# jwcalder/GraphLearningLayer

Hardware: AMD Instinct MI355X
Metric: GLL fwd+bwd calls/sec (base=500,batch=500,d=512,k=10) at 1/2/4/8 GPU (higher is better)
Workload: dtype f32; 1 GPU; ns; base=500, batch=500, d=512, k=10, classes=10, parallelism=dp1, upstream_grad=fixed seeded dL/dU, autograd_thread=caller, collective=none

## Files before the change

graphlearninglayer_amd/_lib.py:

```python
from __future__ import annotations

import ctypes as ct
import os
import threading

HERE = os.path.dirname(os.path.abspath(__file__))
LIB_PATH = os.environ.get("GLL_LIB_PATH") or os.path.join(HERE, "libgll.so")

GLL_OK = 0
GLL_DT_F32, GLL_DT_F64, GLL_DT_I64 = 0, 1, 2
FLAG_CG_GRID = 1
FLAG_CG_PERCOL = 8
FLAG_DIAG_GRID_OVERSUB = 128
FLAG_DIAG_GRID_FAIL = 256
FLAG_CG_ELL = 512
FLAG_CG_VR = 1024
FLAG_GRAD_ROWS = 2048
FLAG_GRAD_CHUNK = 4096
FLAG_GRAM_INLINE = 8192
FLAG_BWD_UNFUSED = 16384
FLAG_KNN_PANEL = 65536
FLAG_D2_F32 = 131072
FLAG_ROW_ORDER_OFF = 262144
KNOB_VR_RV, KNOB_GRID_CAP, KNOB_GRAM_TILE, KNOB_SEL_FORM, KNOB_GRAM_TAIL, KNOB_ROW_PRE = 0, 1, 2, 3, 4, 5
KNOB_GRAD_SPLIT = 6
ST_TINY_EPS, ST_FWD_NONCONV, ST_FWD_ITERS, ST_BWD_NONCONV, ST_BWD_ITERS = 0, 1, 2, 3, 4
ST_KNN_RESCAN = 5
ST_SOLVE_FAILED = 6
ST_GRID_RESCUED = 10
ST_KNN_MERGE = 7
ST_GRAD_SPLIT = 12
ST_NWORDS = 16
K_GRAM, K_SELECT, K_FINALIZE, K_CG, K_EDGE, K_GRAD = range(6)
K_BWD = 6
K_PARAM = 7
K_LOSS = 8
K_COUNT = 9
PG_Y, PG_TAU, PG_EPS = 1, 2, 4
SCORE_NONE, SCORE_ENTROPY, SCORE_L2 = 0, 1, 2
XT_F32, XT_F16, XT_BF16 = 0, 1, 2
UF_NORMALIZE = 1
MAX_D_FEATURES = 4096

EXPORTS = (
    "gll_workspace_bytes", "gll_forward", "gll_backward", "gll_forward_batched",
    "gll_backward_batched", "gll_param_grad_scratch_bytes", "gll_param_grad_batched",
    "gll_ce_head_scratch_bytes", "gll_ce_head_batched", "gll_margin_head_scratch_bytes",
    "gll_margin_head_batched", "gll_graph", "gll_workspace_view",
    "gll_cg_csr_workspace_bytes", "gll_cg_csr", "gll_prof_enable", "gll_prof_read",
    "gll_kernel_name", "gll_strerror", "gll_set_knob", "gll_build_id", "gll_select_route",
    "gll_workspace_solve_view", "gll_workspace_knn_view", "gll_gram_route",
    "gll_features_forward", "gll_features_backward", "gll_features_calls", "gll_fused_plan",
    "gll_objective_head_scratch_bytes", "gll_objective_head_batched",
)


class Problem(ct.Structure):
    _fields_ = [
        ("n", ct.c_int32), ("d", ct.c_int32), ("base", ct.c_int32), ("C", ct.c_int32),
        ("K", ct.c_int32), ("max_iter", ct.c_int32), ("tau", ct.c_float), ("eps", ct.c_float),
        ("rtol", ct.c_float), ("flags", ct.c_int32), ("status_sink", ct.c_void_p),
    ]


class View(ct.Structure):
    _fields_ = [(name, ct.c_void_p) for name in (
        "knn_idx", "knn_d2", "eps", "row_start", "row_len", "col", "w", "d2", "deg", "U32",
        "wadj", "status")]


class SolveView(ct.Structure):
    _fields_ = [(name, ct.c_void_p) for name in ("ucnt", "diag", "rhs", "P", "ell", "vr")] + [
        (name, ct.c_int32) for name in ("SE", "VRM", "Wcap", "RCAP")]


class KnnView(ct.Structure):
    _fields_ = [(name, ct.c_void_p) for name in (
        "D2", "d2_scale", "xhi", "xlo", "xnrm", "pid", "perm")] + [("plane_stride", ct.c_int64)] + [
        (name, ct.c_int32) for name in ("planes", "ldD", "rows", "d2_half", "dp", "order")]


GRAM_ROUTE_WORDS = 9
GRAM_BF3, GRAM_BF3H, GRAM_BF3S, GRAM_BF3W, GRAM_PK, GRAM_PK2 = range(6)

_lock = threading.Lock()
_lib = None


def _declare(lib):
    P = ct.POINTER(Problem)
    vp, i32, sz = ct.c_void_p, ct.c_int, ct.c_size_t
    lib.gll_workspace_bytes.argtypes = [P]
    lib.gll_workspace_bytes.restype = sz
    lib.gll_forward.argtypes = [P, vp, vp, i32, vp, vp, vp]
    lib.gll_forward.restype = i32
    lib.gll_backward.argtypes = [P, vp, vp, i32, vp, vp, i32, vp, vp]
    lib.gll_backward.restype = i32
    lib.gll_forward_batched.argtypes = [P, i32, vp, vp, i32, vp, vp, vp]
    lib.gll_forward_batched.restype = i32
    lib.gll_backward_batched.argtypes = [P, i32, vp, vp, vp, i32, vp, vp]
    lib.gll_backward_batched.restype = i32
    lib.gll_param_grad_scratch_bytes.argtypes = [P, i32]
    lib.gll_param_grad_scratch_bytes.restype = sz
    lib.gll_param_grad_batched.argtypes = [P, i32, vp, i32, vp, vp, vp, vp, vp]
    lib.gll_param_grad_batched.restype = i32
    lib.gll_ce_head_scratch_bytes.argtypes = [P, i32]
    lib.gll_ce_head_scratch_bytes.restype = sz
    lib.gll_ce_head_batched.argtypes = [P, i32, vp, vp, vp, vp, vp, vp, vp, vp, vp]
    lib.gll_ce_head_batched.restype = i32
    lib.gll_margin_head_scratch_bytes.argtypes = [P, i32]
    lib.gll_margin_head_scratch_bytes.restype = sz
    lib.gll_margin_head_batched.argtypes = [P, i32, vp, vp, vp, vp, vp, vp, vp, vp, vp, vp]
    lib.gll_margin_head_batched.restype = i32
    lib.gll_objective_head_scratch_bytes.argtypes = [P, i32]
    lib.gll_objective_head_scratch_bytes.restype = sz
    f64 = ct.c_double
    lib.gll_objective_head_batched.argtypes = [P, i32, vp, vp, f64, f64, f64, vp, vp, vp, vp, vp,
                                               vp, vp, i32, vp, ct.c_int64, vp, vp, vp]
    lib.gll_objective_head_batched.restype = i32
    lib.gll_graph.argtypes = [P, vp, vp, vp]
    lib.gll_graph.restype = i32
    lib.gll_workspace_view.argtypes = [P, vp, ct.POINTER(View)]
    lib.gll_workspace_view.restype = i32
    lib.gll_workspace_solve_view.argtypes = [P, vp, ct.POINTER(SolveView)]
    lib.gll_workspace_solve_view.restype = i32
    lib.gll_workspace_knn_view.argtypes = [P, i32, vp, ct.POINTER(KnnView)]
    lib.gll_workspace_knn_view.restype = i32
    lib.gll_gram_route.argtypes = [P, i32, i32, i32, ct.POINTER(ct.c_int32)]
    lib.gll_gram_route.restype = i32
    lib.gll_cg_csr_workspace_bytes.argtypes = [i32, i32]
    lib.gll_cg_csr_workspace_bytes.restype = sz
    lib.gll_cg_csr.argtypes = [i32, i32, vp, vp, vp, vp, vp, ct.c_float, i32, vp, vp, vp, vp]
    lib.gll_cg_csr.restype = i32
    lib.gll_prof_enable.argtypes = [i32, i32]
    lib.gll_prof_enable.restype = i32
    lib.gll_prof_read.argtypes = [i32, ct.POINTER(ct.c_double), ct.POINTER(ct.c_int)]
    lib.gll_prof_read.restype = i32
    lib.gll_kernel_name.argtypes = [i32]
    lib.gll_kernel_name.restype = ct.c_char_p
    lib.gll_select_route.argtypes = [ct.POINTER(Problem), i32, i32, i32, ct.POINTER(ct.c_int32)]
    lib.gll_select_route.restype = i32
    lib.gll_fused_plan.argtypes = [ct.POINTER(Problem), i32, i32, ct.POINTER(ct.c_int32)]
    lib.gll_fused_plan.restype = i32
    lib.gll_set_knob.argtypes = [i32, i32]
    lib.gll_set_knob.restype = i32
    lib.gll_strerror.argtypes = [i32]
    lib.gll_strerror.restype = ct.c_char_p
    lib.gll_build_id.argtypes = []
    lib.gll_build_id.restype = ct.c_char_p
    lib.gll_features_forward.argtypes = [ct.c_int64, ct.c_int32, vp, i32, i32, vp, vp, vp]
    lib.gll_features_forward.restype = i32
    lib.gll_features_backward.argtypes = [ct.c_int64, ct.c_int32, vp, vp, vp, i32, vp, i32, vp]
    lib.gll_features_backward.restype = i32
    lib.gll_features_calls.argtypes = []
    lib.gll_features_calls.restype = ct.c_int64
    return lib


def build_id() -> str:
    return lib().gll_build_id().decode()


def lib():
    global _lib
    if _lib is None:
        with _lock:
            if _lib is None:
                if not os.path.exists(LIB_PATH):
                    raise RuntimeError(
                        f"{LIB_PATH} is missing: build the HIP extension first "
                        "(python graphlearninglayer_amd/build.py). There is no CPU fallback.")
                _lib = _declare(ct.CDLL(LIB_PATH))
    return _lib


def check(rc: int, what: str):
    if rc != GLL_OK:
        raise RuntimeError(f"{what} failed: {lib().gll_strerror(rc).decode()} (code {rc})")


def kernel_name(kid: int) -> str:
    return lib().gll_kernel_name(kid).decode()
# ... 15 lines not shown
```

graphlearninglayer_amd/csrc/api.hip:

```cpp
#include <atomic>
#include <cstdio>
#include <cstdlib>
#include <mutex>
#include <unordered_map>
#include <vector>

#include "knn_route.h"

namespace gll {

struct ProfState {
    int period[GLL_K_COUNT] = {};
    long count[GLL_K_COUNT] = {};
    bool on[GLL_K_COUNT] = {};
    std::vector<hipEvent_t> pending[GLL_K_COUNT];
    std::vector<hipEvent_t> pool;
    std::mutex mu;
    hipEvent_t get() {
        if (!pool.empty()) {
            hipEvent_t e = pool.back();
            pool.pop_back();
            return e;
        }
        hipEvent_t e;
// ... 415 lines not shown
    out->diag = L.at<float>(ws, L.diag);
    out->rhs = L.at<float>(ws, L.rhs);
    out->P = L.at<float>(ws, L.P);
    out->ell = L.at<int32_t>(ws, L.ell);
    out->vr = L.at<char>(ws, L.vr);
    out->SE = ell_emit(L, 1);
    out->VRM = L.VRM;
    out->Wcap = L.Wcap;
    out->RCAP = L.RCAP;
    return GLL_OK;
}

int gll_workspace_knn_view(const gll_problem* p, int B, void* ws, gll_knn_view* out) {
    int rc = check(p);
    if (rc != GLL_OK) return rc;
    if (B < 1 || B > 65535 || !ws || !out) return GLL_ERR_INVALID_ARG;
    Layout L(*p);
    if (L.PR < L.n && B > 1) return GLL_ERR_UNSUPPORTED;
    Batch bt;
    bt.B = B;
    out->D2 = L.at<float>(ws, L.D2);
    out->d2_scale = L.at<float>(ws, L.d2s);
    out->xhi = L.at<char>(ws, L.xhi);
    out->xlo = L.at<char>(ws, L.xlo);
    out->xnrm = L.at<float>(ws, L.xnrm);
    out->pid = L.at<int32_t>(ws, L.pid);
    out->perm = L.at<int32_t>(ws, L.perm);
    out->plane_stride = int64_t(L.n) * L.ldD;
    out->planes = gram_planes(L, B);
    out->ldD = L.ldD;
    out->rows = L.PR;
    out->d2_half = d2_half(L, bt);
    out->dp = L.dp;
    out->order = locality_order(L, bt);
    return GLL_OK;
}

int gll_gram_route(const gll_problem* p, int B, int x_aligned, int cus,
                   int32_t out[GLL_GRAM_ROUTE_WORDS]) {
    int rc = check(p);
    if (rc != GLL_OK) return rc;
    if (B < 1 || B > 65535 || cus < 1 || !out) return GLL_ERR_INVALID_ARG;
    Layout L(*p);
    if (L.PR < L.n && B > 1) return GLL_ERR_UNSUPPORTED;
    Batch bt;
    bt.B = B;
    const GramRoute rt = gram_route(L, bt, x_aligned && p->d % 4 == 0, cus);
    const int32_t words[GLL_GRAM_ROUTE_WORDS] = {rt.family, rt.vec, rt.planes, rt.presplit, rt.H,
                                                 rt.t256,   rt.tail, rt.sub,   rt.panels};
    for (int q = 0; q < GLL_GRAM_ROUTE_WORDS; ++q) out[q] = words[q];
    return GLL_OK;
}

int gll_cg_csr(int m, int C, const int32_t* row_ptr, const int32_t* col, const float* val,
               const float* b, float* x, float atol, int max_iter, int32_t* iters,
               int32_t* nonconv, void* workspace, void* stream) {
    if (m < 1 || C < 1 || !row_ptr || !col || !val || !b || !x) return GLL_ERR_INVALID_ARG;
    if (m > 2048 && C <= 16) {
        if (!workspace) return GLL_ERR_INVALID_ARG;
        prof_begin(GLL_K_CG, static_cast<hipStream_t>(stream));
        const hipError_t e = launch_cg_grid_csr(m, C, row_ptr, col, val, -1, b, x,
                                                atol, max_iter > 0 ? max_iter : 100000, iters,
                                                nonconv, nullptr,
                                                static_cast<float*>(workspace),
                                                static_cast<hipStream_t>(stream));
        prof_end(GLL_K_CG, static_cast<hipStream_t>(stream));
        if (e != hipErrorNotSupported) return hip_status(e);
    }
    return hip_status(launch_cg_csr(m, C, row_ptr, col, val, b, x, atol,
                                    max_iter > 0 ? max_iter : 100000, iters, nonconv,
                                    static_cast<float*>(workspace),
                                    static_cast<hipStream_t>(stream)));
}

size_t gll_cg_csr_workspace_bytes(int m, int C) {
    const size_t per_col = size_t(5) * m * C, grid = grid_cg_workspace_floats(m, C);
    return (per_col > grid ? per_col : grid) * sizeof(float);
}

int gll_set_knob(int id, int value) {
    if (id < 0 || id >= GLL_KNOB_COUNT || value < 0) return GLL_ERR_INVALID_ARG;
    g_knobs[id].store(value, std::memory_order_relaxed);
    return GLL_OK;
}

int gll_prof_enable(int kid, int period) {
    if (kid < 0 || kid >= GLL_K_COUNT || period < 0) return GLL_ERR_INVALID_ARG;
    std::lock_guard<std::mutex> lk(g_prof.mu);
    g_prof.on[kid] = period > 0;
    g_prof.period[kid] = period > 0 ? period : 1;
    g_prof.count[kid] = 0;
    if (g_armed.kid == kid) g_armed = ArmedLaunch{};
    return GLL_OK;
}

int gll_prof_read(int kid, double* ms_total, int* count) {
    if (kid < 0 || kid >= GLL_K_COUNT || !ms_total || !count) return GLL_ERR_INVALID_ARG;
    std::lock_guard<std::mutex> lk(g_prof.mu);
    auto& v = g_prof.pending[kid];
    double tot = 0.0;
    int cnt = 0;
    for (size_t q = 0; q + 1 < v.size(); q += 2) {
        if (hipEventSynchronize(v[q + 1]) != hipSuccess) return GLL_ERR_HIP;
        float ms = 0.f;
        if (hipEventElapsedTime(&ms, v[q], v[q + 1]) != hipSuccess) return GLL_ERR_HIP;
        tot += ms;
// ... 129 lines not shown
```

graphlearninglayer_amd/csrc/gram.hip:

```cpp
#include "knn_route.h"

namespace gll {

GLL_TRACE_UNIT(knn)

typedef __bf16 bf16x8 __attribute__((ext_vector_type(8)));
typedef __bf16 bf16x4 __attribute__((ext_vector_type(4)));

__device__ __forceinline__ void shift_to_graph(const float* __restrict__& X, float* __restrict__& D2,
                                               int32_t* __restrict__& status,
                                               int32_t* __restrict__& rev_cnt, size_t xs,
                                               size_t wss) {
    X = gshift_br(X, xs);
    D2 = gshift_br(D2, wss);
    status = gshift_br(status, wss);
    rev_cnt = gshift_br(rev_cnt, wss);
}

template <int NT>
__device__ __forceinline__ void reset_call_counters(int32_t* __restrict__ status,
                                                    int32_t* __restrict__ rev_cnt, int n) {
    const int g = bx() * NT + threadIdx.x;
    if (g < kStWords) status[g] = 0;
    for (int q = g; q < n; q += gridDim.x * NT) rev_cnt[q] = 0;
}

__device__ __forceinline__ void mfma3(f32x16& acc, const __bf16* smem_h, int plane, int oa, int ob) {
    const bf16x8 ha = *reinterpret_cast<const bf16x8*>(smem_h + oa);
    const bf16x8 la = *reinterpret_cast<const bf16x8*>(smem_h + plane + oa);
    const bf16x8 hb = *reinterpret_cast<const bf16x8*>(smem_h + ob);
    const bf16x8 lb = *reinterpret_cast<const bf16x8*>(smem_h + plane + ob);
    acc = __builtin_amdgcn_mfma_f32_32x32x16_bf16(la, hb, acc, 0, 0, 0);
    acc = __builtin_amdgcn_mfma_f32_32x32x16_bf16(ha, lb, acc, 0, 0, 0);
    acc = __builtin_amdgcn_mfma_f32_32x32x16_bf16(ha, hb, acc, 0, 0, 0);
}

template <bool H>
__device__ __forceinline__ void dput(float* D2, size_t o, float v, float s) {
    if constexpr (H) reinterpret_cast<_Float16*>(D2)[o] = static_cast<_Float16>(v * s);
    else D2[o] = v;
}
template <bool H>
__device__ __forceinline__ void dput4(float* D2, size_t o, f32x4 v, float s) {
    if constexpr (H) {
        const h16x4 hv = {static_cast<_Float16>(v.x * s), static_cast<_Float16>(v.y * s),
                          static_cast<_Float16>(v.z * s), static_cast<_Float16>(v.w * s)};
        *reinterpret_cast<h16x4*>(reinterpret_cast<_Float16*>(D2) + o) = hv;
    } else {
        *reinterpret_cast<f32x4*>(D2 + o) = v;
    }
}
constexpr int kBP = 256;
constexpr int kMaxCen = 4096;
constexpr int kBS = kBP + 8;

template <int NT = 1024, typename NF>
__device__ __forceinline__ void bf3_epilogue(const f32x16& acc, const float (&sq)[8], float* smem,
                                             float (*sqp)[16], float* nrm, NF nrm_of, int bi,
                                             int bj, int n, float* __restrict__ D2, int ld,
                                             float* __restrict__ Dz) {
    static_assert(NT == 1024 || NT == 512, "bf3_epilogue: 1024- or 512-thread tiles");
    constexpr int KQ = NT / 256;
    constexpr int EP = 4096 / NT;
    constexpr int CPR = 64 / EP;
    const int tid = threadIdx.x;
    const int lane = lane_id();
    const int w = __builtin_amdgcn_readfirstlane(tid >> 6);
    const int r = lane & 31, h = lane >> 5;
    const int qd = w & 3, kq = w >> 2;
    if constexpr (NT == 1024) {
#pragma unroll
        for (int s = 0; s < 8; ++s) {
            const float t = wave_sum_dpp(sq[s]);
            if (lane == 0) sqp[s][w] = t;
        }
    } else {
#pragma unroll
        for (int s = 0; s < 8; ++s) {
            float t = dpp_add<0xB1, 0xf>(sq[s]);
            t = dpp_add<0x4E, 0xf>(t);
            t = dpp_add<0x141, 0xf>(t);
            t = dpp_add<0x140, 0xf>(t);
            t = dpp_add<0x142, 0xa>(t);
            if ((lane & 31) == 31) sqp[s][2 * w + h] = t;
        }
    }
    __syncthreads();
    float* pw = smem + (kq * 4 + qd) * 32 * 33;
#pragma unroll
    for (int e = 0; e < 16; ++e) pw[((e & 3) + 8 * (e >> 2) + 4 * h) * 33 + r] = acc[e];
    if (tid < 128) nrm[tid] = nrm_of(tid);
    __syncthreads();
    const int ti = tid / CPR, tj = EP * (tid % CPR);
    float v[EP];
    {
        const int q = 2 * (ti >> 5) + (tj >> 5), rr = ti & 31;
#pragma unroll
        for (int e = 0; e < EP; ++e) {
            const int cc = (tj & 31) + e;
            float t = 0.f;
#pragma unroll
            for (int k4 = 0; k4 < KQ; ++k4) t += smem[(k4 * 4 + q) * 32 * 33 + rr * 33 + cc];
            v[e] = t;
        }
    }
    __syncthreads();
    float* tile = smem + KQ * 4 * 32 * 33;
#pragma unroll
    for (int e = 0; e < EP; ++e) tile[ti * 65 + tj + e] = nrm[ti] + nrm[64 + tj + e] - 2.f * v[e];
    __syncthreads();
    const int i = bi * 64 + ti;
    if (i < n) {
#pragma unroll
        for (int c = 0; c < EP; c += 4) {
            float o[4];
#pragma unroll
            for (int e = 0; e < 4; ++e) {
                const int jj = tj + c + e;
                o[e] = (bi == bj && jj < ti) ? tile[jj * 65 + ti] : tile[ti * 65 + jj];
            }
            const int j0 = bj * 64 + tj + c;
            float* dst = D2 + size_t(i) * ld + j0;
            float* dz = Dz ? Dz + size_t(i) * ld + j0 : nullptr;
            if (j0 + 4 <= n) {
                __builtin_nontemporal_store(f32x4{o[0], o[1], o[2], o[3]}, reinterpret_cast<f32x4*>(dst));
                if (dz) __builtin_nontemporal_store(f32x4{0.f, 0.f, 0.f, 0.f}, reinterpret_cast<f32x4*>(dz));
            } else {
#pragma unroll
                for (int e = 0; e < 4; ++e)
                    if (j0 + e < n) {
                        dst[e] = o[e];
                        if (dz) dz[e] = 0.f;
                    }
            }
        }
    }
    const int jr = bj * 64 + ti;
    if (bi != bj && jr < n) {
#pragma unroll
        for (int c = 0; c < EP; c += 4) {
            float o[4];
#pragma unroll
            for (int e = 0; e < 4; ++e) o[e] = tile[(tj + c + e) * 65 + ti];
            const int j0 = bi * 64 + tj + c;
            float* dst = D2 + size_t(jr) * ld + j0;
            if (j0 + 4 <= n) {
                __builtin_nontemporal_store(f32x4{o[0], o[1], o[2], o[3]}, reinterpret_cast<f32x4*>(dst));
            } else {
#pragma unroll
                for (int e = 0; e < 4; ++e)
                    if (j0 + e < n) dst[e] = o[e];
            }
        }
    }
}

template <bool VEC>
__global__ __launch_bounds__(1024) void gram_bf3_kernel(const float* __restrict__ X, int n, int d,
                                                        int T, float* __restrict__ D2, int ld,
                                                        int32_t* __restrict__ status,
                                                        int32_t* __restrict__ rev_cnt,
                                                        size_t xs, size_t wss) {
    GLL_TRACE_SCOPE(4);
    GLL_TRACE_PT(10);
    shift_to_graph(X, D2, status, rev_cnt, xs, wss);
    constexpr int kPlane = 128 * kBS;
    __shared__ __attribute__((aligned(16))) __bf16 smem_h[2 * kPlane];
    __shared__ float sqp[8][16];
    __shared__ float nrm[128];
    __shared__ __attribute__((aligned(16))) float cen[kMaxCen];
    float* smem = reinterpret_cast<float*>(smem_h);
    const int tid = threadIdx.x;
    const int lane = lane_id();
    const int w = __builtin_amdgcn_readfirstlane(tid >> 6);
    const int r = lane & 31, h = lane >> 5;
    int bi = 0, rem = xcd_tile(bx(), gridDim.x);
    while (rem >= T - bi) {
        rem -= T - bi;
        ++bi;
    }
    const int bj = bi + rem;
    reset_call_counters<1024>(status, rev_cnt, n);
    const int fo = 4 * lane;
    auto slot_row = [&](int s) {
        const int R = 16 * s + w;
        const int row = (R < 64 ? bi * 64 + R : bj * 64 + R - 64);
        return X + size_t(row < n ? row : n - 1) * d;
    };
    const int nph = (d + kBP - 1) / kBP;
    f32x16 acc;
#pragma unroll
    for (int e = 0; e < 16; ++e) acc[e] = 0.f;
    float sq[8];
#pragma unroll
    for (int s = 0; s < 8; ++s) sq[s] = 0.f;
    const int qd = w & 3, kq = w >> 2;
    const int qa = qd >> 1, qb = qd & 1;

    auto gload = [&](int ph, f32x4 (&v)[8]) {
        const int k = ph * kBP + fo;
#pragma unroll
        for (int s = 0; s < 8; ++s) v[s] = load4_raw<VEC>(slot_row(s), k, d);
    };
    auto phase = [&](int ph, const f32x4 (&v)[8]) {
        const int k = ph * kBP + fo;
        __syncthreads();
        const f32x4 c = *reinterpret_cast<const f32x4*>(cen + ph * kBP + fo);
// ... 62 lines not shown
    const int lane = lane_id();
    const int w = __builtin_amdgcn_readfirstlane(tid >> 6);
    const int r = lane & 31, h = lane >> 5;
    int bi = 0, rem = xcd_tile(bx(), gridDim.x);
    while (rem >= T - bi) {
        rem -= T - bi;
        ++bi;
    }
    const int bj = bi + rem;
    reset_call_counters<512>(status, rev_cnt, n);
    const int fo = 4 * r;
    const f32x4 c = load4_raw<VEC>(X, fo, d);
    f32x4 v[8];
#pragma unroll
    for (int s = 0; s < 8; ++s) {
        const int R = 16 * s + 2 * w + h;
        const int row = R < 64 ? bi * 64 + R : bj * 64 + R - 64;
        v[s] = load4_raw<VEC>(X + size_t(row < n ? row : n - 1) * d, fo, d);
    }
    float sq[8];
#pragma unroll
    for (int s = 0; s < 8; ++s) {
        const f32x4 f = mask4<VEC>(v[s] - c, fo, d);
        sq[s] = f.x * f.x + f.y * f.y + f.z * f.z + f.w * f.w;
        bf16x4 hv, lv;
#pragma unroll
        for (int e = 0; e < 4; ++e) {
            const __bf16 hb = static_cast<__bf16>(f[e]);
            hv[e] = hb;
            lv[e] = static_cast<__bf16>(f[e] - static_cast<float>(hb));
        }
        const int o = (16 * s + 2 * w + h) * kHS + fo;
        *reinterpret_cast<bf16x4*>(smem_h + o) = hv;
        *reinterpret_cast<bf16x4*>(smem_h + kPlane + o) = lv;
    }
    __syncthreads();
    f32x16 acc;
#pragma unroll
    for (int e = 0; e < 16; ++e) acc[e] = 0.f;
    const int qd = w & 3, kq = w >> 2;
    const int qa = qd >> 1, qb = qd & 1;
#pragma unroll
    for (int st = 0; st < 4; ++st) {
        const int kk = 64 * kq + 16 * st + 8 * h;
        const int oa = (32 * qa + r) * kHS + kk, ob = (64 + 32 * qb + r) * kHS + kk;
        mfma3(acc, smem_h, kPlane, oa, ob);
    }
    bf3_epilogue<512>(acc, sq, smem, sqp, nrm, [&](int t) { return sqp[t >> 4][t & 15]; }, bi, bj,
                      n, D2, ld, nullptr);
}

template <bool VEC>
__global__ __launch_bounds__(1024) void gram_bf3s_kernel(const float* __restrict__ X, int n,
                                                         int d, int T, float* __restrict__ D2,
                                                         int ld, size_t plane,
                                                         int32_t* __restrict__ status,
                                                         int32_t* __restrict__ rev_cnt,
                                                         size_t xs, size_t wss) {
    shift_to_graph(X, D2, status, rev_cnt, xs, wss);
    constexpr int kPlane = 128 * kBS;
    __shared__ __attribute__((aligned(16))) __bf16 smem_h[2 * kPlane];
    __shared__ float sqp[8][16];
    __shared__ float nrm[128];
    float* smem = reinterpret_cast<float*>(smem_h);
    const int tid = threadIdx.x;
    const int lane = lane_id();
    const int w = __builtin_amdgcn_readfirstlane(tid >> 6);
    const int r = lane & 31, h = lane >> 5;
    const int b = xcd_tile(bx(), gridDim.x);
    const bool dg = b < T;
    int bi = b, bj = b, half = 0;
    if (!dg) {
        int rem = (b - T) >> 1;
        half = (b - T) & 1;
        bi = 0;
        while (rem >= T - 1 - bi) {
            rem -= T - 1 - bi;
            ++bi;
        }
        bj = bi + 1 + rem;
    }
    reset_call_counters<1024>(status, rev_cnt, n);
    const int fo = 4 * lane;
    f32x4 v[8];
#pragma unroll
    for (int s = 0; s < 8; ++s) {
        const int R = dg ? 16 * (s & 3) + w : 16 * s + w;
        const int row = R < 64 ? bi * 64 + R : bj * 64 + R - 64;
        const int k = (dg ? (s >> 2) : half) * kBP + fo;
        v[s] = load4_raw<VEC>(X + size_t(row < n ? row : n - 1) * d, k, d);
    }
    const f32x4 cen0 = load4_raw<VEC>(X, (dg ? 0 : half) * kBP + fo, d);
    const f32x4 cen1 = load4_raw<VEC>(X, (dg ? 1 : half) * kBP + fo, d);
    float sq[8];
#pragma unroll
    for (int s = 0; s < 8; ++s) {
        const int k = (dg ? (s >> 2) : half) * kBP + fo;
        const f32x4 f = mask4<VEC>(v[s] - (s >= 4 ? cen1 : cen0), k, d);
        sq[s] = f.x * f.x + f.y * f.y + f.z * f.z + f.w * f.w;
        bf16x4 hv, lv;
#pragma unroll
        for (int e = 0; e < 4; ++e) {
            const __bf16 hb = static_cast<__bf16>(f[e]);
            hv[e] = hb;
            lv[e] = static_cast<__bf16>(f[e] - static_cast<float>(hb));
        }
        const int o = (16 * s + w) * kBS + fo;
        *reinterpret_cast<bf16x4*>(smem_h + o) = hv;
        *reinterpret_cast<bf16x4*>(smem_h + kPlane + o) = lv;
    }
    __syncthreads();
    f32x16 acc;
#pragma unroll
    for (int e = 0; e < 16; ++e) acc[e] = 0.f;
    const int qd = w & 3, kq = w >> 2;
    const int qa = qd >> 1, qb = qd & 1;
#pragma unroll
    for (int st = 0; st < 4; ++st) {
        const int kk = 64 * kq + 16 * st + 8 * h;
        if (dg) {
            mfma3(acc, smem_h, kPlane, (32 * qa + r) * kBS + kk, (32 * qb + r) * kBS + kk);
            mfma3(acc, smem_h, kPlane, (64 + 32 * qa + r) * kBS + kk, (64 + 32 * qb + r) * kBS + kk);
        } else {
            mfma3(acc, smem_h, kPlane, (32 * qa + r) * kBS + kk, (64 + 32 * qb + r) * kBS + kk);
        }
    }
    if (dg)
        bf3_epilogue(acc, sq, smem, sqp, nrm,
                     [&](int t) {
                         const int u = t & 63;
                         return sqp[u >> 4][u & 15] + sqp[(u >> 4) + 4][u & 15];
                     },
                     bi, bj, n, D2, ld, D2 + plane);
    else
        bf3_epilogue(acc, sq, smem, sqp, nrm, [&](int t) { return sqp[t >> 4][t & 15]; }, bi, bj,
                     n, D2 + size_t(half) * plane, ld, nullptr);
}

constexpr int kWP = 128;
constexpr int kWS = kWP + 8;

template <bool VEC>
__global__ __launch_bounds__(1024) void gram_bf3w_kernel(const float* __restrict__ X, int n,
                                                         int d, int T, float* __restrict__ D2,
                                                         int ld, int32_t* __restrict__ status,
                                                         int32_t* __restrict__ rev_cnt,
                                                         size_t xs, size_t wss, int r0,
                                                         int pt) {
    shift_to_graph(X, D2, status, rev_cnt, xs, wss);
    constexpr int kPlane = 256 * kWS;
    __shared__ __attribute__((aligned(16))) __bf16 smem_h[2 * kPlane];
    __shared__ float nrm[256];
    __shared__ __attribute__((aligned(16))) float cen[kMaxCen];
    float* smem = reinterpret_cast<float*>(smem_h);
    const int tid = threadIdx.x;
    const int lane = lane_id();
    const int w = __builtin_amdgcn_readfirstlane(tid >> 6);
    const int r = lane & 31, h = lane >> 5;
    int bi = 0, rem = xcd_tile(bx(), gridDim.x), bj;
    if (pt > 0) {
        bi = (r0 >> 7) + rem / T;
        bj = rem % T;
    } else {
        while (rem >= T - bi) {
            rem -= T - bi;
            ++bi;
        }
        bj = bi + rem;
    }
    if (r0 == 0) reset_call_counters<1024>(status, rev_cnt, n);
    const int fo = 4 * (tid & 31);
    const int rs = tid >> 5;
    auto slot_row = [&](int s) {
        const int R = 32 * s + rs;
        const int row = (R < 128 ? bi * 128 + R : bj * 128 + R - 128);
        return X + size_t(row < n ? row : n - 1) * d;
    };
    const int nph = (d + kWP - 1) / kWP;
    const int sa = w >> 2, sb = w & 3;
    f32x16 acc;
#pragma unroll
    for (int e = 0; e < 16; ++e) acc[e] = 0.f;
    float sq = 0.f;

    auto gload = [&](int ph, f32x4 (&v)[8]) {
        const int k = ph * kWP + fo;
#pragma unroll
        for (int q = 0; q < 8; ++q) v[q] = load4_raw<VEC>(slot_row(q), k, d);
    };
// ... 530 lines not shown
        return;
    }
#pragma unroll
    for (int a = 0; a < 2; ++a) {
        const int ti0 = wr * 64 + a * 32;
        const int i0 = bi * 256 + ti0;
        float ni[16];
#pragma unroll
        for (int e = 0; e < 16; ++e) {
            const int i = i0 + (e & 3) + 8 * (e >> 2) + 4 * h;
            ni[e] = nrm[i < n ? i : n - 1];
        }
#pragma unroll
        for (int b = 0; b < 4; ++b) {
            const int tj = wc * 128 + b * 32 + r;
            const int j = bj * 256 + tj;
            if (diag && wc * 128 + b * 32 + 31 < ti0) continue;
            const float nj = nrm[j < n ? j : n - 1];
            float dv[16];
#pragma unroll
            for (int e = 0; e < 16; ++e) dv[e] = ni[e] + nj - 2.f * acc[a][b][e];
#pragma unroll
            for (int e = 0; e < 16; ++e) {
                const int ti = ti0 + (e & 3) + 8 * (e >> 2) + 4 * h;
                const int i = bi * 256 + ti;
                if (i < n && j < n && (!diag || tj >= ti)) dput<H>(D2, size_t(i) * ld + j, dv[e], dsc);
            }
            if (j < n) {
#pragma unroll
                for (int gq = 0; gq < 4; ++gq) {
                    const int ti = ti0 + 8 * gq + 4 * h;
                    const int i = bi * 256 + ti;
                    const size_t o = size_t(j) * ld + i;
                    if (i + 4 <= n && (!diag || tj >= ti + 3)) {
                        dput4<H>(D2, o, f32x4{dv[4 * gq], dv[4 * gq + 1], dv[4 * gq + 2], dv[4 * gq + 3]}, dsc);
                    } else {
#pragma unroll
                        for (int t = 0; t < 4; ++t)
                            if (i + t < n && (!diag || tj >= ti + t)) dput<H>(D2, o + t, dv[4 * gq + t], dsc);
                    }
                }
            }
        }
    }
}

hipError_t launch_gram(const Layout& L, const Batch& bt, void* ws, const float* X, bool vec,
                       hipStream_t s) {
    float* D2 = L.at<float>(ws, L.D2);
    int32_t* st = L.at<int32_t>(ws, L.status);
    int32_t* rc = L.at<int32_t>(ws, L.rev_cnt);
    const GramRoute rt = gram_route(L, bt, vec, device_cus());
    if (rt.panels) return hipErrorInvalidValue;
    prof_begin(GLL_K_GRAM, s);
    switch (rt.family) {
    case kGramBf3s: {
        const int T = (L.n + 63) / 64;
        const dim3 grid(T * T, bt.B);
        const size_t plane = size_t(L.n) * L.ldD;
        launch_k(rt.vec ? gram_bf3s_kernel<true> : gram_bf3s_kernel<false>, grid, 1024, 0, s, X,
                 L.n, L.d, T, D2, L.ldD, plane, st, rc, bt.x, bt.ws);
        prof_end(GLL_K_GRAM, s);
        return launch_status("gram.hip:launch_gram(bf3s)");
    }
    case kGramPk:
    case kGramPk2: {
        __bf16* Ph = L.at<__bf16>(ws, L.xhi);
        __bf16* Pl = L.at<__bf16>(ws, L.xlo);
        float* nrm = L.at<float>(ws, L.xnrm);
        const bool H = rt.H;
        const int T = (L.n + 127) / 128, T2 = (L.n + 255) / 256;
        const int64_t nt2 = int64_t(bt.B) * T2 * (T2 + 1) / 2;
        const int64_t tail = rt.tail;
        prof_span(tail > 0 ? 3 : 2);
        const dim3 sgrid((L.n + 3) / 4, bt.B);
        float* d2s = L.at<float>(ws, L.d2s);
        launch_k(rt.vec ? gram_split_kernel<true> : gram_split_kernel<false>, sgrid, 256, 0, s, X,
                 L.n, L.d, L.dp, Ph, Pl, nrm, st, rc, bt.x, bt.ws);
        if (rt.t256) {
            launch_k(H ? gram_pk2_kernel<true> : gram_pk2_kernel<false>,
                     dim3(unsigned(nt2 - tail)), 512, 0, s, Ph, Pl, nrm, L.n, L.dp, T2, D2,
                     L.ldD, bt.ws, d2s);
            if (tail > 0 && rt.sub == 4)
                launch_k(H ? gram_pk_kernel<true, 128> : gram_pk_kernel<false, 128>,
                         dim3(unsigned(4 * tail)), 256, 0, s, Ph, Pl, nrm, L.n, L.dp, T, D2, L.ldD,
                         bt.ws, d2s, int(nt2 - tail));
            else if (tail > 0)
                launch_k(H ? gram_pk_kernel<true, 64> : gram_pk_kernel<false, 64>,
                         dim3(unsigned(16 * tail)), 256, 0, s, Ph, Pl, nrm, L.n, L.dp,
                         (L.n + 63) / 64, D2, L.ldD, bt.ws, d2s, int(nt2 - tail));
        } else {
            launch_k(H ? gram_pk_kernel<true, 128> : gram_pk_kernel<false, 128>,
                     dim3(unsigned(bt.B * T * (T + 1) / 2)), 256, 0, s, Ph, Pl, nrm, L.n, L.dp, T,
                     D2, L.ldD, bt.ws, d2s, -1);
        }
        prof_end(GLL_K_GRAM, s);
        return launch_status("gram.hip:launch_gram(pk)");
    }
    case kGramBf3w: {
        const int T = (L.n + 127) / 128;
        const dim3 grid(T * (T + 1) / 2, bt.B);
        launch_k(rt.vec ? gram_bf3w_kernel<true> : gram_bf3w_kernel<false>, grid, 1024, 0, s, X,
                 L.n, L.d, T, D2, L.ldD, st, rc, bt.x, bt.ws, 0, 0);
        prof_end(GLL_K_GRAM, s);
        return launch_status("gram.hip:launch_gram(bf3w)");
    }
    case kGramBf3h: {
        const int T64 = (L.n + 63) / 64;
        const dim3 grid(T64 * (T64 + 1) / 2, bt.B);
        launch_k(rt.vec ? gram_bf3h_kernel<true> : gram_bf3h_kernel<false>, grid, 512, 0, s, X,
                 L.n, L.d, T64, D2, L.ldD, st, rc, bt.x, bt.ws);
        prof_end(GLL_K_GRAM, s);
        return launch_status("gram.hip:launch_gram(bf3h)");
    }
// ... 29 lines not shown
```

graphlearninglayer_amd/csrc/knn_route.h:

```cpp
#pragma once

#include "gll_internal.h"

namespace gll {

typedef _Float16 h16x4 __attribute__((ext_vector_type(4)));
typedef __attribute__((address_space(3))) void lds_void;

__device__ __forceinline__ int xcd_tile(int b, int nt) {
    const int x = b & 7, q = b >> 3;
    const int per = nt >> 3, extra = nt & 7;
    return x * per + (x < extra ? x : extra) + q;
}

constexpr int kPK = 64;
constexpr int kPK2 = 32;

inline bool gram_tile256(const Layout& L, const Batch& bt, int T, int T2, int cus) {
    if (knob(GLL_KNOB_GRAM_TILE) > 0) return knob(GLL_KNOB_GRAM_TILE) == 256 && L.dp % kPK2 == 0;
    if (L.dp % kPK2 || L.dp <= 128) return false;
    const int64_t t1 = int64_t(bt.B) * T * (T + 1) / 2, t2 = int64_t(bt.B) * T2 * (T2 + 1) / 2;
    const int64_t r1 = (t1 + cus - 1) / cus, r2 = (t2 + cus - 1) / cus;
    return r2 * 2 * (L.dp / kPK2) * kPK2 < r1 * (L.dp / kPK) * kPK;
}

inline bool presplit_route(const Layout& L, const Batch& bt) {
    const int T = (L.n + 127) / 128;
    return int64_t(bt.B) * T * (T + 1) / 2 >= 256 &&
           !(L.flags & GLL_FLAG_GRAM_INLINE) && (bt.B > 1 || (L.d > 128 && L.n <= 12288)) &&
           gram_planes(L, bt.B) == 1 && L.PR == L.n;
}
inline bool d2_half(const Layout& L, const Batch& bt) {
    return !(L.flags & GLL_FLAG_D2_F32) && bt.B > 1 && presplit_route(L, bt) &&
           L.K - 1 <= kMaxKm1;
}

constexpr int kHP = 128;
enum GramFamily {
    kGramBf3 = 0,
    kGramBf3h = 1,
    kGramBf3s = 2,
    kGramBf3w = 3,
    kGramPk = 4,
    kGramPk2 = 5,
};
struct GramRoute {
    int family;
    int vec;
    int planes;
    int presplit;
    int H;
    int t256;
    int tail;
    int sub;
    int panels;
};
inline GramRoute gram_route(const Layout& L, const Batch& bt, bool vec, int cus) {
    GramRoute r{};
    r.vec = vec;
    r.planes = gram_planes(L, bt.B);
    if (L.PR < L.n) {
        r.family = kGramBf3w;
        r.panels = (L.n + L.PR - 1) / L.PR;
        return r;
    }
// ... 92 lines not shown
```

include/gll.h:

```cpp
#ifndef GLL_H
#define GLL_H

#include <stddef.h>
#include <stdint.h>

#ifdef __cplusplus
extern "C" {
#endif

#define GLL_OK 0
#define GLL_ERR_INVALID_ARG (-1)
#define GLL_ERR_UNSUPPORTED (-2)
#define GLL_ERR_HIP (-3)

#define GLL_DT_F32 0
#define GLL_DT_F64 1
#define GLL_DT_I64 2

#define GLL_ST_TINY_EPS 0
#define GLL_ST_FWD_NONCONV 1
#define GLL_ST_FWD_ITERS 2
#define GLL_ST_BWD_NONCONV 3
#define GLL_ST_BWD_ITERS 4
#define GLL_ST_KNN_RESCAN 5
#define GLL_ST_SOLVE_FAILED 6
#define GLL_ST_KNN_MERGE 7
#define GLL_ST_GRID_RESCUED 10
#define GLL_ST_GRAD_SPLIT 12
#define GLL_ST_NWORDS 16

#define GLL_FLAG_CG_GRID 1
#define GLL_FLAG_CG_PERCOL 8
#define GLL_FLAG_DIAG_GRID_OVERSUB 128
#define GLL_FLAG_DIAG_GRID_FAIL 256
#define GLL_FLAG_CG_ELL 512
#define GLL_FLAG_CG_VR 1024
#define GLL_FLAG_GRAD_ROWS 2048
#define GLL_FLAG_GRAD_CHUNK 4096
#define GLL_FLAG_GRAM_INLINE 8192
#define GLL_FLAG_BWD_UNFUSED 16384
#define GLL_FLAG_KNN_PANEL 65536
#define GLL_FLAG_D2_F32 131072
#define GLL_FLAG_ROW_ORDER_OFF 262144
#define GLL_FLAG_ALL (1 | 8 | 128 | 256 | 512 | 1024 | 2048 | 4096 | 8192 | 16384 | 65536 | \
                      131072 | 262144)

#define GLL_KNOB_VR_RV 0
#define GLL_KNOB_GRID_CAP 1
#define GLL_KNOB_GRAM_TILE 2
#define GLL_KNOB_SEL_FORM 3
#define GLL_KNOB_GRAM_TAIL 4
#define GLL_KNOB_ROW_PRE 5
#define GLL_KNOB_GRAD_SPLIT 6
#define GLL_KNOB_COUNT 7
int gll_set_knob(int knob, int value);

typedef struct gll_problem {
    int32_t n;
    int32_t d;
    int32_t base;
    int32_t C;
    int32_t K;
    int32_t max_iter;
    float tau;
    float eps;
    float rtol;
    int32_t flags;
    int32_t* status_sink;
} gll_problem;

size_t gll_workspace_bytes(const gll_problem* p);

int gll_forward(const gll_problem* p, const float* X, const void* Y, int y_dtype,
                void* workspace, double* U, void* stream);

int gll_backward(const gll_problem* p, const float* X, const void* Y, int y_dtype,
                 void* workspace, const void* gbar, int g_dtype, float* gradX, void* stream);

int gll_forward_batched(const gll_problem* p, int B, const float* X, const void* Y, int y_dtype,
                        void* workspace, double* U, void* stream);
int gll_backward_batched(const gll_problem* p, int B, const float* X, void* workspace,
                         const void* gbar, int g_dtype, float* gradX, void* stream);

#define GLL_PG_Y   1
#define GLL_PG_TAU 2
#define GLL_PG_EPS 4
size_t gll_param_grad_scratch_bytes(const gll_problem* p, int B);
int gll_param_grad_batched(const gll_problem* p, int B, void* workspace, int what,
                           float* gradY, double* grad_tau, double* grad_eps,
                           void* scratch, void* stream);

size_t gll_ce_head_scratch_bytes(const gll_problem* p, int B);
int gll_ce_head_batched(const gll_problem* p, int B, void* workspace, const int64_t* targets,
                        double* loss, float* gbar, double* row_loss, int64_t* pred_label,
                        int64_t* correct, void* scratch, void* stream);

size_t gll_margin_head_scratch_bytes(const gll_problem* p, int B);
int gll_margin_head_batched(const gll_problem* p, int B, void* workspace,
                            const int64_t* other ,
                            double* loss, float* gbar, double* row_margin,
                            int64_t* label, int64_t* second, int64_t* moved,
                            void* scratch, void* stream);

#define GLL_SCORE_NONE    0
#define GLL_SCORE_ENTROPY 1
#define GLL_SCORE_L2      2
size_t gll_objective_head_scratch_bytes(const gll_problem* p, int B);
// ... 9 lines not shown

typedef struct gll_view {
    int32_t* knn_idx;
    float* knn_d2;
    float* eps;
    int32_t* row_start;
    int32_t* row_len;
    int32_t* col;
    float* w;
    float* d2;
    float* deg;
    float* U32;
    float* wadj;
    int32_t* status;
} gll_view;
int gll_workspace_view(const gll_problem* p, void* workspace, gll_view* out);

typedef struct gll_solve_view {
    int32_t* ucnt;
    float* diag;
    float* rhs;
    float* P;
    int32_t* ell;
    void* vr;
    int32_t SE;
    int32_t VRM;
    int32_t Wcap;
    int32_t RCAP;
} gll_solve_view;
int gll_workspace_solve_view(const gll_problem* p, void* workspace, gll_solve_view* out);

typedef struct gll_knn_view {
    void* D2;
    float* d2_scale;
    void* xhi;
    void* xlo;
    float* xnrm;
    int32_t* pid;
    int32_t* perm;
    int64_t plane_stride;
    int32_t planes;
    int32_t ldD;
    int32_t rows;
    int32_t d2_half;
    int32_t dp;
    int32_t order;
} gll_knn_view;
int gll_workspace_knn_view(const gll_problem* p, int B, void* workspace, gll_knn_view* out);

#define GLL_GRAM_ROUTE_WORDS 9
int gll_gram_route(const gll_problem* p, int B, int x_aligned, int cus,
                   int32_t out[GLL_GRAM_ROUTE_WORDS]);

size_t gll_cg_csr_workspace_bytes(int m, int C);
int gll_cg_csr(int m, int C, const int32_t* row_ptr, const int32_t* col, const float* val,
               const float* b, float* x, float atol, int max_iter, int32_t* iters,
               int32_t* nonconv, void* workspace, void* stream);

#define GLL_K_GRAM 0
#define GLL_K_SELECT 1
#define GLL_K_FINALIZE 2
#define GLL_K_CG 3
#define GLL_K_EDGE 4
#define GLL_K_GRAD 5
#define GLL_K_BWD 6
#define GLL_K_PARAM 7
#define GLL_K_LOSS 8
#define GLL_K_COUNT 9
int gll_prof_enable(int kid, int period);
int gll_prof_read(int kid, double* ms_total, int* count);
const char* gll_kernel_name(int kid);

#define GLL_SEL_ROUTE_WORDS 12
int gll_select_route(const gll_problem* p, int B, int x_aligned, int rows,
                     int32_t out[GLL_SEL_ROUTE_WORDS]);

#define GLL_FUSED_PLAN_WORDS 8
int gll_fused_plan(const gll_problem* p, int x_aligned, int capacity,
                   int32_t out[GLL_FUSED_PLAN_WORDS]);

const char* gll_build_id(void);

const char* gll_strerror(int code);

#define GLL_XT_F32 0
#define GLL_XT_F16 1
#define GLL_XT_BF16 2
#define GLL_UF_NORMALIZE 1
int gll_features_forward(int64_t rows, int32_t d, const void* Z, int z_dtype, int flags,
                         float* X, float* rnorm, void* stream);
int gll_features_backward(int64_t rows, int32_t d, const float* gX, const float* X,
                          const float* rnorm, int flags, void* gZ, int z_dtype, void* stream);
int64_t gll_features_calls(void);

#ifdef __cplusplus
}
#endif
#endif
```

Before: 16540 calls/s.

## Replace gram bf3s tile decode with cache-aware host-built tile map

The bf3s Gram kernel now reads its (bi,bj,half,diag) assignment from a host-precomputed packed table passed as a kernel argument, instead of decoding it with a loop. By default the table orders tiles into quadrant groups so that blocks sharing X rows run close together across XCDs; a knob restores the former order. The epilogue now writes off-diagonal tiles directly from registers before the barrier and only uses the LDS transpose for diagonal and mirrored writes. The centroid loads are hoisted ahead of the row loads, and optional trace timestamps are added. The kernel argument grows by 512 bytes, and T is capped at 16.

```diff
diff --git a/graphlearninglayer_amd/_lib.py b/graphlearninglayer_amd/_lib.py
--- a/graphlearninglayer_amd/_lib.py
+++ b/graphlearninglayer_amd/_lib.py
@@ -24,6 +24,7 @@
 FLAG_ROW_ORDER_OFF = 262144
 KNOB_VR_RV, KNOB_GRID_CAP, KNOB_GRAM_TILE, KNOB_SEL_FORM, KNOB_GRAM_TAIL, KNOB_ROW_PRE = 0, 1, 2, 3, 4, 5
 KNOB_GRAD_SPLIT = 6
+KNOB_GRAM_MAP = 7
 ST_TINY_EPS, ST_FWD_NONCONV, ST_FWD_ITERS, ST_BWD_NONCONV, ST_BWD_ITERS = 0, 1, 2, 3, 4
 ST_KNN_RESCAN = 5
 ST_SOLVE_FAILED = 6
@@ -51,7 +52,7 @@
     "gll_kernel_name", "gll_strerror", "gll_set_knob", "gll_build_id", "gll_select_route",
     "gll_workspace_solve_view", "gll_workspace_knn_view", "gll_gram_route",
     "gll_features_forward", "gll_features_backward", "gll_features_calls", "gll_fused_plan",
-    "gll_objective_head_scratch_bytes", "gll_objective_head_batched",
+    "gll_objective_head_scratch_bytes", "gll_objective_head_batched", "gll_gram_tile_map",
 )
 
 
@@ -128,6 +129,8 @@
     lib.gll_workspace_knn_view.restype = i32
     lib.gll_gram_route.argtypes = [P, i32, i32, i32, ct.POINTER(ct.c_int32)]
     lib.gll_gram_route.restype = i32
+    lib.gll_gram_tile_map.argtypes = [i32, ct.POINTER(ct.c_int32)]
+    lib.gll_gram_tile_map.restype = i32
     lib.gll_cg_csr_workspace_bytes.argtypes = [i32, i32]
     lib.gll_cg_csr_workspace_bytes.restype = sz
     lib.gll_cg_csr.argtypes = [i32, i32, vp, vp, vp, vp, vp, ct.c_float, i32, vp, vp, vp, vp]
diff --git a/graphlearninglayer_amd/csrc/api.hip b/graphlearninglayer_amd/csrc/api.hip
--- a/graphlearninglayer_amd/csrc/api.hip
+++ b/graphlearninglayer_amd/csrc/api.hip
@@ -491,6 +491,18 @@
     return GLL_OK;
 }
 
+int gll_gram_tile_map(int T, int32_t* out) {
+    if (T < 1 || T > kGramSMaxT || !out) return GLL_ERR_INVALID_ARG;
+    for (int b = 0; b < T * T; ++b) {
+        const GramUnit u = gram_s_unit(b, T);
+        out[4 * b] = u.bi;
+        out[4 * b + 1] = u.bj;
+        out[4 * b + 2] = u.phase;
+        out[4 * b + 3] = u.diag;
+    }
+    return GLL_OK;
+}
+
 int gll_cg_csr(int m, int C, const int32_t* row_ptr, const int32_t* col, const float* val,
                const float* b, float* x, float atol, int max_iter, int32_t* iters,
                int32_t* nonconv, void* workspace, void* stream) {
diff --git a/graphlearninglayer_amd/csrc/gram.hip b/graphlearninglayer_amd/csrc/gram.hip
--- a/graphlearninglayer_amd/csrc/gram.hip
+++ b/graphlearninglayer_amd/csrc/gram.hip
@@ -3,6 +3,15 @@
 namespace gll {
 
 GLL_TRACE_UNIT(knn)
+#ifdef GLL_TRACE
+#define GLL_TRACE_WG(i)                                                                      \
+    do {                                                                                     \
+        if (threadIdx.x == 0 && blockIdx.x < 256 && blockIdx.y == 0)                         \
+            g_wg[256 * (i) + blockIdx.x] = __builtin_amdgcn_s_memrealtime();                 \
+    } while (0)
+#else
+#define GLL_TRACE_WG(i) do {} while (0)
+#endif
 
 typedef __bf16 bf16x8 __attribute__((ext_vector_type(8)));
 typedef __bf16 bf16x4 __attribute__((ext_vector_type(4)));
@@ -104,35 +113,46 @@
             v[e] = t;
         }
     }
+    GLL_TRACE_WG(4);
+    float* tile = smem + KQ * 4 * 32 * 33;
+    float dv[EP];
+#pragma unroll
+    for (int e = 0; e < EP; ++e) {
+        dv[e] = nrm[ti] + nrm[64 + tj + e] - 2.f * v[e];
+        tile[ti * 65 + tj + e] = dv[e];
+    }
+    auto store4 = [&](int row, int j0, const float (&o)[4], float* __restrict__ Dzz) {
+        float* dst = D2 + size_t(row) * ld + j0;
+        float* dz = Dzz ? Dzz + size_t(row) * ld + j0 : nullptr;
+        if (j0 + 4 <= n) {
+            __builtin_nontemporal_store(f32x4{o[0], o[1], o[2], o[3]}, reinterpret_cast<f32x4*>(dst));
+            if (dz) __builtin_nontemporal_store(f32x4{0.f, 0.f, 0.f, 0.f}, reinterpret_cast<f32x4*>(dz));
+        } else {
+#pragma unroll
+            for (int e = 0; e < 4; ++e)
+                if (j0 + e < n) {
+                    dst[e] = o[e];
+                    if (dz) dz[e] = 0.f;
+                }
+        }
+    };
+    const int i = bi * 64 + ti;
+    if (bi != bj && i < n) {
+#pragma unroll
+        for (int c = 0; c < EP; c += 4)
+            store4(i, bj * 64 + tj + c, {dv[c], dv[c + 1], dv[c + 2], dv[c + 3]}, Dz);
+    }
     __syncthreads();
-    float* tile = smem + KQ * 4 * 32 * 33;
-#pragma unroll
-    for (int e = 0; e < EP; ++e) tile[ti * 65 + tj + e] = nrm[ti] + nrm[64 + tj + e] - 2.f * v[e];
-    __syncthreads();
-    const int i = bi * 64 + ti;
-    if (i < n) {
+    if (bi == bj && i < n) {
 #pragma unroll
         for (int c = 0; c < EP; c += 4) {
             float o[4];
 #pragma unroll
             for (int e = 0; e < 4; ++e) {
                 const int jj = tj + c + e;
-                o[e] = (bi == bj && jj < ti) ? tile[jj * 65 + ti] : tile[ti * 65 + jj];
-            }
-            const int j0 = bj * 64 + tj + c;
-            float* dst = D2 + size_t(i) * ld + j0;
-            float* dz = Dz ? Dz + size_t(i) * ld + j0 : nullptr;
-            if (j0 + 4 <= n) {
-                __builtin_nontemporal_store(f32x4{o[0], o[1], o[2], o[3]}, reinterpret_cast<f32x4*>(dst));
-                if (dz) __builtin_nontemporal_store(f32x4{0.f, 0.f, 0.f, 0.f}, reinterpret_cast<f32x4*>(dz));
-            } else {
-#pragma unroll
-                for (int e = 0; e < 4; ++e)
-                    if (j0 + e < n) {
-                        dst[e] = o[e];
-                        if (dz) dz[e] = 0.f;
-                    }
-            }
+                o[e] = jj < ti ? tile[jj * 65 + ti] : tile[ti * 65 + jj];
+            }
+            store4(i, bj * 64 + tj + c, o, Dz);
         }
     }
     const int jr = bj * 64 + ti;
@@ -142,17 +162,10 @@
             float o[4];
 #pragma unroll
             for (int e = 0; e < 4; ++e) o[e] = tile[(tj + c + e) * 65 + ti];
-            const int j0 = bi * 64 + tj + c;
-            float* dst = D2 + size_t(jr) * ld + j0;
-            if (j0 + 4 <= n) {
-                __builtin_nontemporal_store(f32x4{o[0], o[1], o[2], o[3]}, reinterpret_cast<f32x4*>(dst));
-            } else {
-#pragma unroll
-                for (int e = 0; e < 4; ++e)
-                    if (j0 + e < n) dst[e] = o[e];
-            }
-        }
-    }
+            store4(jr, bi * 64 + tj + c, o, nullptr);
+        }
+    }
+    GLL_TRACE_WG(5);
 }
 
 template <bool VEC>
@@ -321,7 +334,8 @@
 
 template <bool VEC>
 __global__ __launch_bounds__(1024) void gram_bf3s_kernel(const float* __restrict__ X, int n,
-                                                         int d, int T, float* __restrict__ D2,
+                                                         int d, const GramSMap map,
+                                                         float* __restrict__ D2,
                                                          int ld, size_t plane,
                                                          int32_t* __restrict__ status,
                                                          int32_t* __restrict__ rev_cnt,
@@ -336,21 +350,16 @@
     const int lane = lane_id();
     const int w = __builtin_amdgcn_readfirstlane(tid >> 6);
     const int r = lane & 31, h = lane >> 5;
-    const int b = xcd_tile(bx(), gridDim.x);
-    const bool dg = b < T;
-    int bi = b, bj = b, half = 0;
-    if (!dg) {
-        int rem = (b - T) >> 1;
-        half = (b - T) & 1;
-        bi = 0;
-        while (rem >= T - 1 - bi) {
-            rem -= T - 1 - bi;
-            ++bi;
-        }
-        bj = bi + 1 + rem;
-    }
+    const uint32_t unit = gram_s_packed(map, bx());
+    const bool dg = unit >> 9 & 1;
+    const int bi = unit & 15, bj = unit >> 4 & 15;
+    const int half = unit >> 8 & 1;
+    GLL_TRACE_WG(0);
     reset_call_counters<1024>(status, rev_cnt, n);
     const int fo = 4 * lane;
+    const f32x4 cen0 = load4_raw<VEC>(X, (dg ? 0 : half) * kBP + fo, d);
+    const f32x4 cen1 = load4_raw<VEC>(X, (dg ? 1 : half) * kBP + fo, d);
+    __builtin_amdgcn_sched_barrier(0);
     f32x4 v[8];
 #pragma unroll
     for (int s = 0; s < 8; ++s) {
@@ -359,8 +368,10 @@
         const int k = (dg ? (s >> 2) : half) * kBP + fo;
         v[s] = load4_raw<VEC>(X + size_t(row < n ? row : n - 1) * d, k, d);
     }
-    const f32x4 cen0 = load4_raw<VEC>(X, (dg ? 0 : half) * kBP + fo, d);
-    const f32x4 cen1 = load4_raw<VEC>(X, (dg ? 1 : half) * kBP + fo, d);
+#ifdef GLL_TRACE
+    if (w == 0) asm volatile("s_waitcnt vmcnt(0)" ::: "memory");
+    GLL_TRACE_WG(1);
+#endif
     float sq[8];
 #pragma unroll
     for (int s = 0; s < 8; ++s) {
@@ -378,7 +389,9 @@
         *reinterpret_cast<bf16x4*>(smem_h + o) = hv;
         *reinterpret_cast<bf16x4*>(smem_h + kPlane + o) = lv;
     }
+    GLL_TRACE_WG(2);
     __syncthreads();
+    GLL_TRACE_WG(7);
     f32x16 acc;
 #pragma unroll
     for (int e = 0; e < 16; ++e) acc[e] = 0.f;
@@ -394,6 +407,7 @@
             mfma3(acc, smem_h, kPlane, (32 * qa + r) * kBS + kk, (64 + 32 * qb + r) * kBS + kk);
         }
     }
+    GLL_TRACE_WG(3);
     if (dg)
         bf3_epilogue(acc, sq, smem, sqp, nrm,
                      [&](int t) {
@@ -404,6 +418,10 @@
     else
         bf3_epilogue(acc, sq, smem, sqp, nrm, [&](int t) { return sqp[t >> 4][t & 15]; }, bi, bj,
                      n, D2 + size_t(half) * plane, ld, nullptr);
+#ifdef GLL_TRACE
+    if (w == 0) asm volatile("s_waitcnt vmcnt(0)" ::: "memory");
+    GLL_TRACE_WG(6);
+#endif
 }
 
 constexpr int kWP = 128;
@@ -1040,6 +1058,7 @@
     int32_t* rc = L.at<int32_t>(ws, L.rev_cnt);
     const GramRoute rt = gram_route(L, bt, vec, device_cus());
     if (rt.panels) return hipErrorInvalidValue;
+    if (rt.family == kGramBf3s && (L.n + 63) / 64 > kGramSMaxT) return hipErrorInvalidValue;
     prof_begin(GLL_K_GRAM, s);
     switch (rt.family) {
     case kGramBf3s: {
@@ -1047,7 +1066,7 @@
         const dim3 grid(T * T, bt.B);
         const size_t plane = size_t(L.n) * L.ldD;
         launch_k(rt.vec ? gram_bf3s_kernel<true> : gram_bf3s_kernel<false>, grid, 1024, 0, s, X,
-                 L.n, L.d, T, D2, L.ldD, plane, st, rc, bt.x, bt.ws);
+                 L.n, L.d, gram_s_map(T, gram_s_former()), D2, L.ldD, plane, st, rc, bt.x, bt.ws);
         prof_end(GLL_K_GRAM, s);
         return launch_status("gram.hip:launch_gram(bf3s)");
     }
diff --git a/graphlearninglayer_amd/csrc/knn_route.h b/graphlearninglayer_amd/csrc/knn_route.h
--- a/graphlearninglayer_amd/csrc/knn_route.h
+++ b/graphlearninglayer_amd/csrc/knn_route.h
@@ -7,10 +7,78 @@
 typedef _Float16 h16x4 __attribute__((ext_vector_type(4)));
 typedef __attribute__((address_space(3))) void lds_void;
 
-__device__ __forceinline__ int xcd_tile(int b, int nt) {
+__host__ __device__ __forceinline__ int xcd_tile(int b, int nt) {
     const int x = b & 7, q = b >> 3;
     const int per = nt >> 3, extra = nt & 7;
     return x * per + (x < extra ? x : extra) + q;
+}
+
+struct GramUnit {
+    int bi, bj;
+    int phase;
+    int diag;
+};
+constexpr int kGramSMaxT = 16;
+struct GramSMap {
+    uint32_t w[kGramSMaxT * kGramSMaxT / 2];
+};
+__host__ __device__ __forceinline__ uint32_t gram_s_packed(const GramSMap& m, int b) {
+    return (m.w[b >> 1] >> (16 * (b & 1))) & 0xffffu;
+}
+
+inline void gram_s_sequence(int T, bool former, GramUnit* seq) {
+    int q = 0;
+    auto tri = [&](int lo, int hi, int ph) {
+        for (int i = lo; i < hi; ++i)
+            for (int j = i + 1; j < hi; ++j) seq[q++] = GramUnit{i, j, ph, 0};
+    };
+    auto dia = [&](int lo, int hi) {
+        for (int i = lo; i < hi; ++i) seq[q++] = GramUnit{i, i, 0, 1};
+    };
+    auto rect = [&](int r0, int r1, int c0, int c1, int ph) {
+        for (int i = r0; i < r1; ++i)
+            for (int j = c0; j < c1; ++j) seq[q++] = GramUnit{i, j, ph, 0};
+    };
+    if (former) {
+        dia(0, T);
+        for (int i = 0; i < T; ++i)
+            for (int j = i + 1; j < T; ++j)
+                for (int ph = 0; ph < 2; ++ph) seq[q++] = GramUnit{i, j, ph, 0};
+        return;
+    }
+    const int h = (T + 1) / 2;
+    const int ha = (h + 1) / 2, hb = h + (T - h + 1) / 2;
+    dia(0, ha), tri(0, h, 0), dia(ha, h), tri(0, h, 1);
+    dia(h, hb), tri(h, T, 0), dia(hb, T), tri(h, T, 1);
+    rect(0, ha, h, T, 0), rect(0, ha, h, T, 1);
+    rect(ha, h, h, T, 0), rect(ha, h, h, T, 1);
+}
+
+inline const GramSMap& gram_s_map(int T, bool former) {
+    struct Tables {
+        GramSMap m[2][kGramSMaxT + 1];
+        Tables() : m{} {
+            GramUnit seq[kGramSMaxT * kGramSMaxT];
+            for (int f = 0; f < 2; ++f)
+                for (int t = 1; t <= kGramSMaxT; ++t) {
+                    gram_s_sequence(t, f == 1, seq);
+                    for (int b = 0; b < t * t; ++b) {
+                        const GramUnit& u = seq[xcd_tile(b, t * t)];
+                        const uint32_t p = uint32_t(u.bi) | uint32_t(u.bj) << 4 |
+                                           uint32_t(u.phase) << 8 | uint32_t(u.diag) << 9;
+                        m[f][t].w[b >> 1] |= p << (16 * (b & 1));
+                    }
+                }
+        }
+    };
+    static const Tables tabs;
+    return tabs.m[former ? 1 : 0][T];
+}
+inline bool gram_s_former() { return knob(GLL_KNOB_GRAM_MAP) == 1; }
+
+inline GramUnit gram_s_unit(int b, int T) {
+    const uint32_t p = gram_s_packed(gram_s_map(T, gram_s_former()), b);
+    return GramUnit{int(p & 15), int(p >> 4 & 15), int(p >> 8 & 1), int(p >> 9 & 1)};
 }
 
 constexpr int kPK = 64;
diff --git a/include/gll.h b/include/gll.h
--- a/include/gll.h
+++ b/include/gll.h
@@ -52,7 +52,8 @@
 #define GLL_KNOB_GRAM_TAIL 4
 #define GLL_KNOB_ROW_PRE 5
 #define GLL_KNOB_GRAD_SPLIT 6
-#define GLL_KNOB_COUNT 7
+#define GLL_KNOB_GRAM_MAP 7
+#define GLL_KNOB_COUNT 8
 int gll_set_knob(int knob, int value);
 
 typedef struct gll_problem {
@@ -168,6 +169,8 @@
 int gll_gram_route(const gll_problem* p, int B, int x_aligned, int cus,
                    int32_t out[GLL_GRAM_ROUTE_WORDS]);
 
+int gll_gram_tile_map(int T, int32_t* out);
+
 size_t gll_cg_csr_workspace_bytes(int m, int C);
 int gll_cg_csr(int m, int C, const int32_t* row_ptr, const int32_t* col, const float* val,
                const float* b, float* x, float atol, int max_iter, int32_t* iters,
```

After: 16700 calls/s, median of 6. About the same (+1.0%).
